# UbiquityRobotics/fiducials

Hardware: AMD Instinct MI355X
Metric: frames/sec @1920x1080 20-marker (aruco detect + pose hot path) (higher is better)
Workload: dtype u8

## Files before the change

fiducials_amd/csrc/fid_api.hip:

```cpp
#include "fid_kernels.hip"

#include <math.h>
#include <stdio.h>
#include <stdlib.h>
#include <string.h>

#include <new>
#include <string>
#include <vector>

namespace {

enum { ST_GRAY = 0, ST_THRESH, ST_STARTS, ST_PROBE, ST_WALK, ST_APPROX, ST_SORT, ST_NEAR, ST_RESOLVE, ST_IDENT, ST_FILTER, ST_SUBPIX, ST_POSE, ST_SEEDWALK,
       ST_SEEDLESS, ST_COUNT };
const char *const kStageNames[ST_COUNT] = {"to_gray", "threshold", "find_starts", "walk_probe", "walk_full", "approx", "sort_cands",
                                           "near", "resolve", "identify", "filter_markers", "subpix", "pose", "seed_walk", "seedless_chain"};

constexpr int TX = 128, TY = 32, NT = 256;
constexpr int THRW_NT = 512, THRW_WT = 16;
static_assert(THRW_NT * THRW_WT >= 8191, "k_threshold_wide: a row per workgroup");

}

struct fid_ctx {
// ... 429 lines not shown
    const int gstride = to_gray ? W : stride;
    const long long gfstride = to_gray ? (long long)W * H : fstride;
    const uint8_t *gray = to_gray ? c->d_gray : d_src;
    set_geometry(c, W, H, gstride, F);
    if (c->wait_ev) {
        HIPCHK(c, hipStreamWaitEvent(st0, c->wait_ev, 0));
        c->wait_ev = nullptr;
    }
    if (c->d_seedhash) {
        if (++c->seed_gen > 1023) {
            HIPCHK(c, hipMemsetAsync(c->d_seedhash, 0, (size_t)c->lim.max_batch * c->seed_hash_cap * sizeof(unsigned long long), st0));
            c->seed_gen = 1;
        }
        c->P.seedGen = c->seed_gen;
    }
    if (c->masks_W != W || c->masks_H != H || c->masks_S != c->P.nscales) {
        HIPCHK(c, hipMemsetAsync(c->d_masks, 0, c->masks_bytes, st0));
        c->masks_W = W;
        c->masks_H = H;
        c->masks_S = c->P.nscales;
    }
    layout_results(c, F);
    if (!c->res_precleared) HIPCHK(c, hipMemsetAsync(c->d_res, 0, c->res_clear_bytes, st0));
    c->res_precleared = false;
    c->piece_chain = c->pieces > 1 && !c->chained && !c->host_feed && !c->from_host_call && !c->whole_border_walk && c->sub_frames <= 0 &&
                     F >= 32 * c->pieces && c->stagger == 0;
    const SubPlan plan = plan_sub_batches(c, F);
    const int nsub = plan.nsub;
    const bool chainp = c->piece_chain;
    c->last_nsub = nsub;
    {
        const fid_status rcs = ensure_streams(c, nsub, F);
        if (rcs != FID_OK) return rcs;
    }
    if (nsub > 1) HIPCHK(c, hipEventRecord(c->fork_ev, st0));
    bool tail_recorded = false;
    auto sub_phase = [&](int sb, int phase) -> fid_status {
        const int f0 = plan.f0[sb], Fs = plan.f0[sb + 1] - f0;
        hipStream_t st = nsub > 1 ? c->sub_stream[chainp ? (sb & 1) : sb] : st0;
        if (nsub > 1 && phase == 0) HIPCHK(c, hipStreamWaitEvent(st, c->fork_ev, 0));
        if (chainp && phase == 0 && sb > 0) HIPCHK(c, hipStreamWaitEvent(st, c->fs_done[sb - 1], 0));
        if (c->host_feed && phase == 0) HIPCHK(c, hipStreamWaitEvent(st, c->in_ready[sb], 0));
        if (nsub > 1 && phase == 0 && c->stagger > 0 && sb >= c->stagger) HIPCHK(c, hipStreamWaitEvent(st, c->walk_done[sb - c->stagger], 0));
        DevParams P = c->P;
        P.nframes = Fs;
        const size_t MC = (size_t)P.maxCands, MM = (size_t)P.maxMarkers;
        const uint8_t *g = gray + (long long)f0 * gfstride;
        uint32_t *masks = c->d_masks + (size_t)f0 * P.nscales * P.TR * P.TC * MT_ROWS;
        uint2 *starts = c->d_starts + (size_t)f0 * P.maxStarts, *surv1 = c->d_surv1 + (size_t)f0 * P.maxStarts,
              *surv = c->d_surv + (size_t)f0 * P.maxStarts;
        uint4 *contours = c->d_contours + (size_t)f0 * P.maxContours;
        uint32_t *tab = c->d_ckpts + (size_t)f0 * 2 * P.maxContours * chunk_tab_pitch(P);
        uint32_t *pool = c->d_pool + (size_t)f0 * P.maxChunks * CKW;
        DevCounts *counts = c->d_counts + f0;
        DevCand *cands = c->d_cands + f0 * MC, *sorted = c->d_sorted + f0 * MC, *filtered = c->d_filtered + f0 * MC;
        uint32_t *nearb = c->d_near + f0 * MC * (MC / 32);
        DevIdent *ident = c->d_ident + f0 * MC;
        fid_marker *pre = c->d_pre + f0 * MM, *markers = c->d_markers + f0 * MM;
        unsigned *worklist = c->d_worklist + f0 * MC, *nwork = c->d_nwork + sb;
        hipEvent_t *ev = c->sub_ev[sb];
        auto mark = [&](int idx) {
            if (c->profile) (void)hipEventRecord(ev[idx], st);
        };
        auto chain_point = [&](int pt) {
            if (sb == nsub - 1 && !tail_recorded && !c->blocking && c->chain_at <= pt) {
                (void)hipEventRecord(c->tail_ev, st);
                tail_recorded = true;
            }
        };
      if (phase == 0) {
        mark(0);
        if (to_gray && (int)enc <= FID_ENC_RGBA8)
            hipLaunchKernelGGL(k_to_gray, dim3(2048), dim3(256), 0, st, d_src + (long long)f0 * fstride, stride, fstride, (int)enc,
                               c->d_gray + (size_t)f0 * W * H, W, H, Fs);
        else if (to_gray)
            hipLaunchKernelGGL(k_raw_to_gray, dim3((W + 255) / 256, (H + 3) / 4, Fs), dim3(64, 4), 0, st, d_src + (long long)f0 * fstride, stride,
                               fstride, (int)enc, c->d_gray + (size_t)f0 * W * H, W, H);
        mark(ST_GRAY + 1);
        {
            bool node_table = P.nscales == 13;
            for (int i = 0; i < P.nscales && node_table; i++) node_table = P.win[i] == 3 + 4 * i;
            if (node_table) {
                const int cols = 64 * c->thr_nw, strips = (W + cols - 1) / cols;
                int RS = c->thr_rows;
                if (RS <= 0) {
                    int segs = (1536 + strips * Fs - 1) / (strips * Fs);
                    const int maxsegs = (H + 63) / 64;
                    segs = segs < 1 ? 1 : (segs > maxsegs ? maxsegs : segs);
                    RS = (H + segs - 1) / segs;
                }
                RS = (RS + 3) & ~3;
                dim3 grid(strips, (H + RS - 1) / RS, Fs);
                if (c->thr_nw == 5 && c->thr_split) launch_thr_stream<5, true>(grid, st, g, gfstride, masks, P, RS, c->thr_xcd);
                else if (c->thr_nw == 5) launch_thr_stream<5, false>(grid, st, g, gfstride, masks, P, RS, c->thr_xcd);
                else if (c->thr_split) launch_thr_stream<3, true>(grid, st, g, gfstride, masks, P, RS, c->thr_xcd);
                else launch_thr_stream<3, false>(grid, st, g, gfstride, masks, P, RS, c->thr_xcd);
            } else if (P.rmax > 40) {
                int bands = (512 + Fs - 1) / Fs;
                const int maxb = (H + 15) / 16;
                bands = bands < 1 ? 1 : (bands > maxb ? maxb : bands);
                const int BH = (H + bands - 1) / bands;
                const size_t lds = (size_t)(W + 1 + THRW_NT / 64) * sizeof(unsigned long long);
                fid_launch_log("k_threshold_wide", THRW_NT, lds);
                hipLaunchKernelGGL((k_threshold_wide<THRW_NT, THRW_WT>), dim3((H + BH - 1) / BH, 1, Fs), dim3(THRW_NT), lds, st, g, gfstride,
                                   masks, P, BH);
            } else {
                int R = P.rmax, RW = TX + 2 * R, RH = TY + 2 * R, PT = (RW + 1) | 1;
                size_t lds = (size_t)(RH + 1) * PT * sizeof(uint32_t);
                dim3 grid((W + TX - 1) / TX, (H + TY - 1) / TY, Fs);
                hipLaunchKernelGGL((k_threshold<TX, TY, NT>), grid, dim3(NT), lds, st, g, gfstride, masks, P);
            }
        }
        mark(ST_THRESH + 1);
      }
        long long k2blocks;
        {
            long long groups = (long long)P.nscales * P.TR * ((P.WW + 15) / 16);
            k2blocks = (groups + 7) / 8;
            if (k2blocks > 256) k2blocks = 256;
        }
      if (phase == 0) {
        if (!c->whole_border_walk) {
            hipLaunchKernelGGL(k_find_starts<true>, dim3((unsigned)k2blocks, Fs), dim3(256), 0, st, masks, starts, counts, c->d_global,
                               c->d_seedq + f0 * (size_t)P.maxContours, P);
            mark(ST_STARTS + 1);
            if (nsub > 1) HIPCHK(c, hipEventRecord(c->fs_done[sb], st));
            chain_point(0);
        }
        return FID_OK;
      }
        if (!c->whole_border_walk && nsub > 1 && c->fs_barrier && !chainp)
            for (int o = 0; o < nsub; o++)
                if (o != sb) HIPCHK(c, hipStreamWaitEvent(st, c->fs_done[o], 0));
        int wb = c->walk_blocks > 0 ? c->walk_blocks : (3072 / WALK_WAVES + Fs - 1) / Fs;
        const int wcap = c->walk_blocks_cap > 0 ? c->walk_blocks_cap : (Fs <= 2 ? 256 : 64);
        wb = wb < 2 ? 2 : (wb > wcap ? wcap : wb);
        const int gm = Fs >= 16 ? 1 : 16 / Fs;
        const int wb2 = wb > 1 ? wb / 2 : 1;
        const int cap1 = pts_cap_first(P);
        const size_t lds1 = k_approx_lds_bytes(cap1);
        const size_t lds2 = k_approx_lds_bytes(P.maxPerim + 1);
        if (c->whole_border_walk) {
            hipLaunchKernelGGL(k_find_starts<false>, dim3((unsigned)k2blocks, Fs), dim3(256), 0, st, masks, starts, counts, c->d_global,
                               (uint2 *)nullptr, P);
            mark(ST_STARTS + 1);
            hipLaunchKernelGGL((k_probe<PROBE0_STEPS, 0>), dim3(64 * gm, Fs), dim3(256), 0, st, masks, starts, surv1, counts, c->d_global, P);
            hipLaunchKernelGGL((k_probe<PROBE1_STEPS, 1>), dim3(16 * gm, Fs), dim3(256), 0, st, masks, surv1, surv, counts, c->d_global, P);
            mark(ST_PROBE + 1);
            hipLaunchKernelGGL(k_walk_full<0>, dim3(wb, Fs), dim3(64 * WALK_WAVES), 0, st, masks, surv, contours, tab, pool, (DevSegC *)nullptr,
                               (DevPend *)nullptr, counts, c->d_global, P);
            mark(ST_WALK + 1);
            fid_launch_log("k_approx", 64, (size_t)(lds1));
            hipLaunchKernelGGL(k_approx, dim3(128 * gm, Fs), dim3(64), lds1, st, contours, tab, pool, cands, counts, P, cap1, 0,
                               (const uint32_t *)nullptr, (const uint32_t *)nullptr);
            fid_launch_log("k_approx", 64, (size_t)(lds2));
            hipLaunchKernelGGL(k_approx, dim3(16 * gm, Fs), dim3(64), lds2, st, contours, tab, pool, cands, counts, P,
                               P.maxPerim + 1, 1, (const uint32_t *)nullptr, (const uint32_t *)nullptr);
            mark(ST_APPROX + 1);
        } else {
            const size_t MCn = (size_t)P.maxContours;
            DevSegC *segs = c->d_segs + f0 * MCn;
            DevPend *pend = c->d_pend + f0 * MCn;
            uint2 *seedq = c->d_seedq + f0 * MCn;
            unsigned long long *seedhash = c->d_seedhash + (size_t)f0 * P.seedHashCap;
            uint4 *wres = c->d_wres + f0 * MCn, *cinfo = c->d_cinfo + f0 * MCn;
            uint32_t *cbase = c->d_cbase + f0 * MCn;
            uint32_t *dense = c->d_dense + (size_t)f0 * P.maxChunks * (CK / 4);
            hipStream_t sa = c->aux_stream[chainp ? (sb & 1) : sb];
            HIPCHK(c, hipEventRecord(c->aux_fork[sb], st));
            HIPCHK(c, hipStreamWaitEvent(sa, c->aux_fork[sb], 0));
            int swb = c->sw_blocks > 0 ? c->sw_blocks : (1024 / SW_WAVES + Fs - 1) / Fs;
            swb = swb < 2 ? 2 : (swb > 4 * wcap ? 4 * wcap : swb);
            uint4 *recs = c->d_recs + 2 * f0 * MCn;
            const int cpb = c->copy_blocks > 0 ? c->copy_blocks : 256;
            if (c->profile) (void)hipEventRecord(ev[14], st);
            hipLaunchKernelGGL(k_seed_walk, dim3(swb, Fs), dim3(64 * SW_WAVES), 0, st, masks, seedq, tab, pool, segs, counts, c->d_global, P);
            if (c->profile) (void)hipEventRecord(ev[15], st);
            mark(ST_PROBE + 1);
            chain_point(1);
            if (c->profile) (void)hipEventRecord(ev[16], sa);
            hipStream_t si = (nsub == 1 && Fs <= 16 && c->idx_stream) ? c->idx_stream : sa;
            if (si != sa) HIPCHK(c, hipStreamWaitEvent(si, c->aux_fork[sb], 0));
            hipLaunchKernelGGL(k_seed_index, dim3(8 * gm, Fs), dim3(256), 0, si, seedq, seedhash, counts, P);
            HIPCHK(c, hipEventRecord(c->aux_idx[sb], si));
            if (c->probe_refill0 && gm == 1)
                hipLaunchKernelGGL((k_probe_refill<PROBE0_STEPS, 0>), dim3(c->probe_refill0, Fs), dim3(256), 0, sa, masks, starts, surv1, counts, c->d_global, P,
                                   (const uint4 *)c->d_probe_tables);
            else
                hipLaunchKernelGGL((k_probe_lut<PROBE0_STEPS, 0>), dim3(64 * gm, Fs), dim3(256), 0, sa, masks, starts, surv1, counts, c->d_global, P,
                                   (const uint4 *)c->d_probe_tables);
            if (c->probe_refill && gm == 1)
                hipLaunchKernelGGL((k_probe_refill<PROBE1_STEPS, 1>), dim3(c->probe_refill, Fs), dim3(256), 0, sa, masks, surv1, surv, counts, c->d_global, P,
                                   (const uint4 *)c->d_probe_tables);
            else
                hipLaunchKernelGGL((k_probe_lut<PROBE1_STEPS, 1>), dim3(16 * gm, Fs), dim3(256), 0, sa, masks, surv1, surv, counts, c->d_global, P,
                                   (const uint4 *)c->d_probe_tables);
            const int wb3 = c->walk2_div > 0 ? (wb / c->walk2_div > 0 ? wb / c->walk2_div : 1) : wb2;
            hipLaunchKernelGGL(k_walk_full<2>, dim3(wb3, Fs), dim3(64 * WALK_WAVES), 0, sa, masks, surv, wres, tab, pool, segs, pend, counts,
                               c->d_global, P);
            if (si != sa) HIPCHK(c, hipStreamWaitEvent(sa, c->aux_idx[sb], 0));
            hipLaunchKernelGGL(k_seg_cycles<0>, dim3(8 * gm, Fs), dim3(64), 0, sa, seedq, segs, pend, wres, contours, cinfo, cbase,
                               recs, counts, c->d_global, P, 1, 0);
            hipLaunchKernelGGL(k_seg_copy, dim3(cpb / 4 > 0 ? cpb / 4 : 1, Fs), dim3(256), 0, sa, recs, tab, pool, dense, counts, P, 1);
            fid_launch_log("k_approx", 64, (size_t)(lds1));
            hipLaunchKernelGGL(k_approx, dim3(32 * gm, Fs), dim3(64), lds1, sa, contours, tab, pool, cands, counts, P, cap1, 0,
                               dense, cbase, 2);
            fid_launch_log("k_approx", 64, (size_t)(lds2));
            hipLaunchKernelGGL(k_approx, dim3(8 * gm, Fs), dim3(64), lds2, sa, contours, tab, pool, cands, counts, P,
                               P.maxPerim + 1, 1, dense, cbase, 2);
            if (c->profile) (void)hipEventRecord(ev[17], sa);
            HIPCHK(c, hipEventRecord(c->aux_join[sb], sa));
            HIPCHK(c, hipStreamWaitEvent(st, c->aux_idx[sb], 0));
            hipLaunchKernelGGL(k_seg_link2, dim3(16 * gm, Fs), dim3(256), 0, st, seedq, segs, seedhash, counts, P);
            const int scb = Fs <= 2 ? (int)((P.maxContours + 63) / 64 < 4096 ? (P.maxContours + 63) / 64 : 4096) : 32 * gm * c->light_x;
            if (Fs <= 2)
                hipLaunchKernelGGL(k_seg_cycles<48>, dim3(scb, Fs), dim3(64), 0, st, seedq, segs, pend, wres, contours, cinfo, cbase,
                                   recs, counts, c->d_global, P, 0, getenv("FID_NO_SEGC_WARM") ? 0 : 1);
            else
                hipLaunchKernelGGL(k_seg_cycles<0>, dim3(scb, Fs), dim3(64), 0, st, seedq, segs, pend, wres, contours, cinfo, cbase,
                                   recs, counts, c->d_global, P, 0, 0);
            hipLaunchKernelGGL(k_seg_copy, dim3(cpb, Fs), dim3(256), 0, st, recs, tab, pool, dense, counts, P, 0);
            mark(ST_WALK + 1);
            chain_point(2);
            fid_launch_log("k_approx", 64, (size_t)(lds1));
            hipLaunchKernelGGL(k_approx, dim3(128 * gm, Fs), dim3(64), lds1, st, contours, tab, pool, cands, counts, P, cap1, 0,
                               dense, cbase, 1);
            fid_launch_log("k_approx", 64, (size_t)(lds2));
            hipLaunchKernelGGL(k_approx, dim3(16 * gm, Fs), dim3(64), lds2, st, contours, tab, pool, cands, counts, P,
                               P.maxPerim + 1, 1, dense, cbase, 1);
            mark(ST_APPROX + 1);
            chain_point(3);
            if (chainp) {
                HIPCHK(c, hipEventRecord(c->front_done[sb], st));
                HIPCHK(c, hipStreamWaitEvent(sa, c->front_done[sb], 0));
                st = sa;
            } else {
                HIPCHK(c, hipStreamWaitEvent(st, c->aux_join[sb], 0));
            }
        }
        if (nsub > 1 && c->stagger > 0) HIPCHK(c, hipEventRecord(c->walk_done[sb], st));
        chain_point(4);
        float4 *cmeta = c->d_cmeta + f0 * MC;
        fid_launch_log("k_sort_cands", 256, (size_t)(MC * 8));
        hipLaunchKernelGGL(k_sort_cands, dim3(Fs, (c->light_x > 1 || Fs < 16) ? 16 : 1), dim3(256), MC * 8, st, cands, sorted, cmeta, counts, P);
        mark(ST_SORT + 1);
        hipLaunchKernelGGL(k_near, dim3(32 * gm * c->light_x, Fs), dim3(256), 0, st, sorted, cmeta, nearb, counts, P);
        mark(ST_NEAR + 1);
        {
            const size_t lds = (size_t)c->resolve_lds_kb * 1024;
            const int near_words = c->resolve_serial ? 0 : (int)((lds - 3 * MC * 4) / 4);
            fid_launch_log("k_resolve", 1024, (size_t)(lds));
            hipLaunchKernelGGL(k_resolve, dim3(Fs), dim3(1024), lds, st, sorted, nearb, filtered, counts, worklist, nwork, P, near_words, c->d_global,
                               c->resolve_reg_max);
        }
        mark(ST_RESOLVE + 1);
        chain_point(5);
        {
            int SZ = (P.markerSize + 2 * P.borderBits) * P.cellSize;
            fid_launch_log("k_identify", 64, (size_t)((size_t)SZ * SZ));
            hipLaunchKernelGGL(k_identify, dim3(c->tail_grid > 0 ? c->tail_grid : 256 * 4), dim3(64), (size_t)SZ * SZ, st, g, gfstride, filtered, worklist, nwork,
                               c->d_dict, ident, c->d_bits + f0 * MC * (size_t)(P.markerSize + 2 * P.borderBits) * (P.markerSize + 2 * P.borderBits), P);
        }
        mark(ST_IDENT + 1);
        fid_launch_log("k_filter_markers", 64, (size_t)((size_t)c->filter_lds * sizeof(fid_marker)));
        hipLaunchKernelGGL(k_filter_markers, dim3(Fs), dim3(64), (size_t)c->filter_lds * sizeof(fid_marker), st, filtered, ident, pre, counts, P,
                           c->d_filter_scratch + f0 * MC, c->filter_lds, c->d_accsrc + f0 * MC, c->d_mksrc + f0 * MM);
        mark(ST_FILTER + 1);
        {
            long long items = (long long)Fs * P.maxMarkers * 4;
            const long long bcap = c->tail_grid > 0 ? 4LL * c->tail_grid : 256 * 16;
            int blocks = (int)(items < bcap ? items : bcap);
            if (P.refine == 2)
                hipLaunchKernelGGL(k_refine_contour, dim3(P.maxMarkers < 64 ? P.maxMarkers : 64, Fs), dim3(64), 0, st, (const fid_marker *)pre, markers,
                                   (const int *)(c->d_mksrc + f0 * MM), (const DevCand *)filtered,
                                   (const uint32_t *)(c->d_dense ? c->d_dense + (size_t)f0 * P.maxChunks * (CK / 4) : nullptr), (const uint32_t *)tab,
                                   (const uint32_t *)pool, counts, P);
            else if (P.subpixWin <= 7)
                hipLaunchKernelGGL(k_subpix<7>, dim3(blocks), dim3(64), 0, st, g, gfstride, pre, markers, counts, c->d_subpix_mask, P);
            else
                hipLaunchKernelGGL(k_subpix<SP_MAXWIN_MAX>, dim3(blocks), dim3(64), 0, st, g, gfstride, pre, markers, counts, c->d_subpix_mask, P);
        }
        mark(ST_SUBPIX + 1);
        if (c->pose_cam_valid) {
            PoseCam cam;
            for (int i = 0; i < 9; i++) cam.K[i] = c->pose_K[i];
            for (int i = 0; i < 5; i++) cam.D[i] = c->pose_D[i];
            cam.fiducial_len = c->pose_len;
            int blocks = (Fs * P.maxMarkers + 7) / 8;
            blocks = blocks < 1 ? 1 : (blocks > 256 * 16 ? 256 * 16 : blocks);
            if (c->profile) (void)hipEventRecord(ev[18], st);
            hipLaunchKernelGGL(k_pose, dim3(blocks), dim3(64), 0, st, (const fid_marker *)markers, (const int *)&counts[0].nmark,
                               (int)(sizeof(DevCounts) / sizeof(int)), (const double *)nullptr, Fs, P.maxMarkers, cam, c->d_poses + f0 * MM);
            if (c->profile) (void)hipEventRecord(ev[19], st);
        }
        chain_point(99);
        if (nsub > 1) {
            HIPCHK(c, hipEventRecord(c->sub_done[sb], st));
            if (!chainp) HIPCHK(c, hipStreamWaitEvent(st0, c->sub_done[sb], 0));
        }
        return FID_OK;
    };
    if (chainp) {
        for (int sb = 0; sb < nsub; sb++)
            for (int phase = 0; phase < 2; phase++) {
                const fid_status rcs = sub_phase(sb, phase);
                if (rcs != FID_OK) return rcs;
            }
        for (int sb = 0; sb < nsub; sb++) HIPCHK(c, hipStreamWaitEvent(st0, c->sub_done[sb], 0));
    } else {
        for (int phase = 0; phase < 2; phase++)
            for (int sb = 0; sb < nsub; sb++) {
                const fid_status rcs = sub_phase(sb, phase);
                if (rcs != FID_OK) return rcs;
            }
    }
    hipStream_t st = st0;
    const DevParams &P = c->P;
    HIPCHK(c, hipGetLastError());
    c->pose_done = false;
    c->map_done = false;
    const bool map_ahead = c->map_n > 0 && c->map_cam_valid;
    if (map_ahead) {
        map_pose_launch(c, st, c->d_markers, &c->d_counts[0].nmark, (int)(sizeof(DevCounts) / sizeof(int)), P.maxMarkers, F, c->map_K, c->map_D, c->d_mposes);
        HIPCHK(c, hipGetLastError());
    }
    HIPCHK(c, hipMemcpyAsync(c->h_res, c->d_res, c->pose_cam_valid ? c->res_poses_end : c->res_markers_end, hipMemcpyDeviceToHost, st));
    if (map_ahead) HIPCHK(c, hipMemcpyAsync(c->h_mposes, c->d_mposes, sizeof(fid_map_pose_out) * (size_t)F, hipMemcpyDeviceToHost, st));
    c->last_frames = F;
    c->last_W = W;
    c->last_H = H;
    c->last_gray = gray;
    c->last_gfstride = gfstride;
    c->pend = {d_src, F, W, H, stride, fstride, enc};
    c->in_flight = true;
    c->chained = false;
    c->wait_ev = nullptr;
    c->wait_copy_ev = nullptr;
    c->fed_from_host = false;
    return FID_OK;
}

fid_status run_detect(fid_ctx *c, const uint8_t *d_src, int F, int W, int H, int stride, long long fstride, fid_encoding enc,
                      fid_marker *out, int cap_per_frame, int *n_per_frame);

fid_status finish_detect(fid_ctx *c, fid_marker *out, int cap_per_frame, int *n_per_frame)
{
    const DevParams &P = c->P;
    const int F = c->pend.F;
    c->in_flight = false;
    HIPCHK(c, hipStreamSynchronize(c->stream));
    c->pose_done = c->pose_cam_valid;
    c->map_done = c->map_n > 0 && c->map_cam_valid;
    if (c->profile) {
        for (int i = 0; i < ST_COUNT; i++) c->stage_ms[i] = 0.f;
        for (int sb = 0; sb < c->last_nsub; sb++)
            for (int i = 0; i <= ST_SUBPIX; i++) {
                float ms = 0.f;
                if (hipEventElapsedTime(&ms, c->sub_ev[sb][i], c->sub_ev[sb][i + 1]) == hipSuccess) c->stage_ms[i] += ms;
            }
        if (!c->whole_border_walk)
            for (int sb = 0; sb < c->last_nsub; sb++) {
                float ms = 0.f;
                if (hipEventElapsedTime(&ms, c->sub_ev[sb][14], c->sub_ev[sb][15]) == hipSuccess) c->stage_ms[ST_SEEDWALK] += ms;
                if (hipEventElapsedTime(&ms, c->sub_ev[sb][16], c->sub_ev[sb][17]) == hipSuccess) c->stage_ms[ST_SEEDLESS] += ms;
                if (c->pose_cam_valid && hipEventElapsedTime(&ms, c->sub_ev[sb][18], c->sub_ev[sb][19]) == hipSuccess) c->stage_ms[ST_POSE] += ms;
            }
    }
#ifdef FID_DEBUG_STATS
    {
        const unsigned long long *d = c->h_global->dbg;
        fprintf(stderr, "walk stats: ranges %llu iters %llu ckpts %llu (forced %llu) active-lanes/iter %.1f cyc/range %.0f ckpt-cyc/range %.0f wait-cyc/range %.0f\n",
                d[7], d[0], d[1], d[5], d[0] ? (double)d[2] / d[0] : 0., d[7] ? (double)d[6] / d[7] : 0., d[7] ? (double)d[3] / d[7] : 0.,
                d[7] ? (double)d[4] / d[7] : 0.);
        fprintf(stderr, "walk waves %llu: total cyc avg %.0f max %llu; own queue dry at avg %.0f max %llu\n", d[12],
                d[12] ? (double)d[8] / d[12] : 0., d[9], d[12] ? (double)d[10] / d[12] : 0., d[11]);
        fprintf(stderr, "walk longest %llu steps, total steps %llu\n", d[13], d[14]);
        fprintf(stderr, "resolve (frame 0, n %llu, %llu label rounds) cycles: load %llu label %llu count %llu components %llu places %llu move %llu\n", d[31] >> 32,
                d[31] & 0xffffffffull, d[25], d[26], d[27], d[28], d[29], d[30]);
        if (d[1])
            fprintf(stderr, "checkpoint cycles: wait %.0f activate %.0f retire %.0f hand-out %.0f chunks %.0f refill %.0f; lanes at a checkpoint: need %.1f loading %.1f final %.1f idle %.1f\n",
                    (double)d[4] / d[1], (double)d[16] / d[1], (double)d[17] / d[1], (double)d[18] / d[1], (double)d[19] / d[1], (double)d[20] / d[1],
                    (double)d[21] / d[1], (double)d[22] / d[1], (double)d[23] / d[1], (double)d[24] / d[1]);
// ... 859 lines not shown
```

fiducials_amd/csrc/fid_kernels.hip:

```cpp
#include <hip/hip_runtime.h>
#include <stdint.h>
#include <float.h>
#include <limits.h>

#include <type_traits>
#include <utility>

#include "fid_device.h"
#include "../../include/fid_abi.h"

#define WAVE 64

__device__ __forceinline__ int lane_id() { return threadIdx.x & (WAVE - 1); }

__device__ __forceinline__ unsigned long long ballot64(int pred) { return __ballot(pred); }

#define FID_DPP(OLD, V, CTRL, RMASK) __builtin_amdgcn_update_dpp((OLD), (V), (CTRL), (RMASK), 0xf, false)
#define FID_DPP_SCAN_STEPS(STEP) STEP(0x111, 0xf) STEP(0x112, 0xf) STEP(0x114, 0xf) STEP(0x118, 0xf) STEP(0x142, 0xa) STEP(0x143, 0xc)

__device__ __forceinline__ int wave_iscan(int v)
{
#define S_(C, M) v += FID_DPP(0, v, C, M);
    FID_DPP_SCAN_STEPS(S_)
#undef S_
// ... 2379 lines not shown
#ifdef FID_DEBUG_STATS
    if (lane == 0) {
        atomicAdd(&G->dbg[0], d_iters);
        atomicAdd(&G->dbg[1], d_ckpts);
        atomicAdd(&G->dbg[2], d_active);
        atomicAdd(&G->dbg[3], d_ckcyc);
        atomicAdd(&G->dbg[6], (unsigned long long)(__builtin_readcyclecounter() - d_t0));
        atomicAdd(&G->dbg[7], 1ull);
        for (int k = 0; k < 4; k++) atomicAdd(&G->dbg[21 + k], d_lanes[k]);
    }
#endif
}

__global__ __launch_bounds__(256) void k_seg_link2(const uint2 *__restrict__ seedq, DevSegC *__restrict__ segs,
                                                    const unsigned long long *__restrict__ seedhash, const DevCounts *__restrict__ counts,
                                                    const DevParams P)
{
    const int f = blockIdx.y;
    unsigned ns = (unsigned)counts[f].nseeds;
    ns = ns < (unsigned)P.maxContours ? ns : (unsigned)P.maxContours;
    const unsigned long long *fsh = seedhash + (long long)f * P.seedHashCap;
    const uint2 *fsq = seedq + (long long)f * P.maxContours;
    DevSegC *fsg = segs + (long long)f * P.maxContours;
    for (unsigned i = blockIdx.x * blockDim.x + threadIdx.x; i < ns; i += gridDim.x * blockDim.x) {
        if (fsg[i].n == SEG_INVALID) continue;
        const unsigned nx = seedhash_find(fsh, P.seedHashCap, P.seedGen, seedhash_key(fsg[i].next_key, (int)(fsq[i].x >> 27)));
        if (nx < ns) {
            fsg[i].next_idx = nx;
            fsg[nx].linked = 1u;
        }
    }
}

template <unsigned SC_HOPS>
__global__ __launch_bounds__(64) void k_seg_cycles(const uint2 *__restrict__ seedq, const DevSegC *__restrict__ segs,
                                                    const DevPend *__restrict__ pend, const uint4 *__restrict__ wres,
                                                    uint4 *__restrict__ contours, uint4 *__restrict__ cinfo, uint32_t *__restrict__ cbase,
                                                    uint4 *__restrict__ recs, DevCounts *__restrict__ counts, DevGlobal *__restrict__ G,
                                                    const DevParams P, int part, int warm)
{
    __shared__ uint2 s_hops[SC_HOPS ? SC_HOPS : 1][SC_HOPS ? 64 : 1];
    const int f = blockIdx.y;
    const int lane = lane_id();
    unsigned ns = (unsigned)counts[f].nseeds, nv = (unsigned)counts[f].nsurv;
    ns = ns < (unsigned)P.maxContours ? ns : (unsigned)P.maxContours;
    nv = nv < (unsigned)P.maxContours ? nv : (unsigned)P.maxContours;
    const unsigned lcap = (unsigned)P.maxContours / 2u, rcap = (unsigned)P.maxContours;
    const uint2 *fsq = seedq + (long long)f * P.maxContours;
    const DevSegC *fsg = segs + (long long)f * P.maxContours;
    const DevPend *fpd = pend + (long long)f * P.maxContours;
    uint4 *fco = contours + (long long)f * P.maxContours + (part ? lcap : 0u);
    uint4 *fci = cinfo + (long long)f * P.maxContours + (part ? lcap : 0u);
    uint32_t *fcb = cbase + (long long)f * P.maxContours + (part ? lcap : 0u);
    uint4 *frc = recs + (long long)f * 2 * P.maxContours + (part ? rcap : 0u);
    unsigned *cnt_slots = (unsigned *)(part ? &counts[f].ncontours2 : &counts[f].ncontours);
    unsigned *cnt_recs = (unsigned *)(part ? &counts[f].nrec2 : &counts[f].nrec);
    const unsigned dcap = (unsigned)P.maxChunks * CK;
    const unsigned W2 = (unsigned)P.W + 2u;
    const unsigned ibeg = part ? ns : 0u, iend = part ? ns + nv : ns;
    if (warm && !part) {
        const unsigned nlines = (ns * (unsigned)sizeof(DevSegC) + 127u) >> 7, nx = (gridDim.x + 7u) >> 3;
        unsigned acc = 0;
        for (unsigned k = (blockIdx.x >> 3) * 64u + (unsigned)lane; k < nlines; k += nx * 64u)
            acc += *reinterpret_cast<const volatile uint32_t *>(reinterpret_cast<const char *>(fsg) + (size_t)k * 128u);
        asm volatile("" ::"v"(acc));
    }
    for (unsigned i0 = ibeg + blockIdx.x * 64; i0 < iend; i0 += gridDim.x * 64) {
        const unsigned i = i0 + lane;
        int accept = 0, hole = 0;
        unsigned L = 0, key = 0, hops = 0, pos = 0, n0 = 0, nx0 = SEG_INVALID;
        uint2 st = make_uint2(0u, 0u);
        if (i < ns) {
            const DevSegC s = fsg[i];
            if (s.n != SEG_INVALID && s.n != 0u && s.linked && (s.ko & s.kh) != 0xffffffffu) {
                bool co = s.ko != 0xffffffffu, ch = s.kh != 0xffffffffu, closed = false;
                unsigned KO = s.ko, KH = s.kh, cur = s.next_idx;
                L = s.n;
                hops = 1;
                while (cur != SEG_INVALID) {
                    if (cur == i) {
                        closed = true;
                        break;
                    }
                    DevSegC r;
                    {
                        const uint4 q = reinterpret_cast<const uint4 *>(fsg + cur)[0];
                        r.next_idx = q.x;
                        r.n = q.y;
                        r.ko = q.z;
                        r.kh = q.w;
                    }
                    if (r.n == SEG_INVALID || r.n == 0u) break;
                    co = co && !(r.ko < s.ko);
                    ch = ch && !(r.kh < s.kh);
                    if (!co && !ch) break;
                    KO = r.ko < KO ? r.ko : KO;
                    KH = r.kh < KH ? r.kh : KH;
                    L += r.n;
                    if (SC_HOPS && hops - 1u < SC_HOPS) s_hops[hops - 1u][lane] = make_uint2(cur, r.n);
                    hops++;
                    if (L > (unsigned)P.maxPerim) break;
                    cur = r.next_idx;
                }
                if (closed && L >= (unsigned)P.minPerim && L <= (unsigned)P.maxPerim) {
                    if (co && KO < KH) {
                        accept = 1;
                        hole = 0;
                        key = s.ko;
                        pos = s.pos & 0xffffu;
                    } else if (ch && KH < KO) {
                        accept = 1;
                        hole = 1;
                        key = s.kh;
                        pos = s.pos >> 16;
                    }
                }
                if (accept) {
                    n0 = s.n;
                    nx0 = s.next_idx;
                    const unsigned ky = key / W2, kx = key - ky * W2;
                    st = make_uint2((kx - 1u - (unsigned)hole) | ((ky - 1u) << 16), (uint32_t)f | ((fsq[i].x >> 27) << 16) | ((uint32_t)hole << 24));
                }
            }
        } else if (i < iend) {
            const unsigned j = i - ns;
            if (!fpd[j].p) {
                const uint4 w = wres[(long long)f * P.maxContours + j];
                if (w.z) {
                    st = make_uint2(w.x, w.y);
                    L = w.z;
                    key = w.w;
                    accept = 2;
                }
            }
        }
        const unsigned long long mk = ballot64(accept);
        if (mk) {
            const unsigned myL = accept ? (L + 7u) & ~7u : 0u, myR = accept == 1 ? hops + 1u : (accept == 2 ? 1u : 0u);
            const unsigned sL = wave_iscan_dpp(myL), sR = wave_iscan_dpp(myR);
            const unsigned totL = (unsigned)__builtin_amdgcn_readlane((int)sL, 63), totR = (unsigned)__builtin_amdgcn_readlane((int)sR, 63);
            unsigned bslot = 0, bdense = 0, brec = 0;
            if (lane == 63) {
                bslot = atomicAdd(cnt_slots, (unsigned)__popcll(mk));
                bdense = atomicAdd((unsigned *)&counts[f].ndense, totL);
                brec = atomicAdd(cnt_recs, totR);
            }
            bslot = (unsigned)__builtin_amdgcn_readlane((int)bslot, 63);
            bdense = (unsigned)__builtin_amdgcn_readlane((int)bdense, 63);
            brec = (unsigned)__builtin_amdgcn_readlane((int)brec, 63);
            const unsigned idx = bslot + (unsigned)__popcll(mk & ((1ull << lane) - 1ull));
            if (accept) {
                if (idx < lcap) {
                    fco[idx] = make_uint4(st.x, st.y, L, key);
                    fci[idx] = make_uint4(i, pos, nx0, 0u);
                    const unsigned dst0 = bdense + sL - myL;
                    unsigned rec = brec + sR - myR;
                    if (dst0 + L > dcap || rec + myR > rcap) {
                        atomicOr(&G->overflow, 8u);
                        fcb[idx] = SEG_INVALID;
                    } else if (accept == 2) {
                        fcb[idx] = dst0;
                        frc[rec] = make_uint4((unsigned)P.maxContours + (i - ns), dst0, L, REC_NO_CHUNK);
                    } else {
                        fcb[idx] = dst0;
                        const unsigned ck0 = fsg[i].chunk0;
                        frc[rec++] = make_uint4(i, dst0, (n0 - pos) | (pos << 16), ck0);
                        unsigned off = n0 - pos, cur = nx0;
                        {
                            const unsigned noted = !SC_HOPS ? 0u : (hops - 1u < SC_HOPS ? hops - 1u : SC_HOPS);
                            for (unsigned h = 0; h < noted; h++) {
                                const uint2 e = s_hops[h][lane];
                                frc[rec++] = make_uint4(e.x, dst0 + off, e.y, fsg[e.x].chunk0);
                                off += e.y;
                                cur = e.x;
                            }
                            if (noted) cur = hops - 1u > noted ? fsg[cur].next_idx : i;
                        }
                        while (cur != i && cur != SEG_INVALID && off < L) {
                            const uint2 q = reinterpret_cast<const uint2 *>(fsg + cur)[0];
                            frc[rec++] = make_uint4(cur, dst0 + off, q.y, fsg[cur].chunk0);
                            off += q.y;
                            cur = q.x;
                        }
                        frc[rec++] = make_uint4(i, dst0 + off, pos, ck0);
                        for (; rec < brec + sR; rec++) frc[rec] = make_uint4(0u, 0u, 0u, 0u);
                    }
                } else {
                    atomicOr(&G->overflow, 2u);
                }
            }
        }
    }
}

#define K4_SHORT_PTS 2048
#define K4_MAX_RAW 9
#define K4_STACK 16
__device__ __host__ inline int pts_cap_first(const DevParams &P) { return P.maxPerim < K4_SHORT_PTS ? P.maxPerim : K4_SHORT_PTS; }
inline size_t k_approx_lds_bytes(int pts_cap) { return (size_t)((pts_cap + 7) & ~7) * sizeof(uint32_t); }

__global__ __launch_bounds__(64) void k_approx(const uint4 *__restrict__ contours, const uint32_t *__restrict__ chunk_tab,
                                                const uint32_t *__restrict__ pool, DevCand *__restrict__ cands,
                                                DevCounts *__restrict__ counts, const DevParams P, int pts_cap, int second_pass,
                                                const uint32_t *__restrict__ dense, const uint32_t *__restrict__ cbase, int part = 0)
{
    extern __shared__ __attribute__((aligned(16))) uint32_t pts[];
    __shared__ int2 stack[K4_STACK];
    __shared__ int dst[2 * 16];
    const int lane = lane_id();
    const int f = blockIdx.y;
    unsigned n = (unsigned)(dense ? (part == 2 ? counts[f].ncontours2 : counts[f].ncontours) : counts[f].nsurv);
    n = n < (unsigned)P.maxStarts ? n : (unsigned)P.maxStarts;
    n = n < (unsigned)P.maxContours ? n : (unsigned)P.maxContours;
    const unsigned loff = part == 2 ? (unsigned)P.maxContours / 2u : 0u;
    if (part) n = n < (unsigned)P.maxContours / 2u ? n : (unsigned)P.maxContours / 2u;
    const int W = P.W, H = P.H;
    const uint4 *fco = contours + (long long)f * P.maxContours + loff;
    const uint32_t *fpool = pool;
    for (unsigned cb = blockIdx.x; cb < n; cb += gridDim.x * 64) {
      const unsigned myci = cb + (unsigned)lane * gridDim.x;
      uint4 mine = make_uint4(0u, 0u, 0u, 0u);
      if (myci < n) mine = fco[myci];
      int take = mine.z != 0;
      if (second_pass) take = take && (int)mine.z > pts_cap_first(P);
      else take = take && (int)mine.z <= pts_cap;
      unsigned long long todo = ballot64(take);
      while (todo) {
        const int src = __ffsll((long long)todo) - 1;
        todo &= todo - 1;
        const unsigned ci = cb + (unsigned)src * gridDim.x;
        uint4 c;
        c.x = (unsigned)__builtin_amdgcn_readlane((int)mine.x, src);
        c.y = (unsigned)__builtin_amdgcn_readlane((int)mine.y, src);
        c.z = (unsigned)__builtin_amdgcn_readlane((int)mine.z, src);
        c.w = (unsigned)__builtin_amdgcn_readlane((int)mine.w, src);
        const int count = (int)c.z;
        const int x0 = c.x & 0xffff, y0 = c.x >> 16;
        const int s = (c.y >> 16) & 0xff, hole = (c.y >> 24) & 1;
        __syncthreads();
        uint32_t pref = 0x80000000u | ci;
        if (dense) {
            const uint32_t cb0 = cbase[(long long)f * P.maxContours + loff + ci];
            if (cb0 == SEG_INVALID) continue;
            pref = cb0;
            const uint8_t *src = reinterpret_cast<const uint8_t *>(dense) + (long long)f * P.maxChunks * CK + cb0;
            uint32_t base = c.x;
            for (int k0 = 0; k0 < count; k0 += 512) {
                const int k = k0 + 8 * lane;
                uint2 w = make_uint2(0u, 0u);
                if (k < count) w = *reinterpret_cast<const uint2 *>(src + k);
                base = codes8_to_points(pts, k, count, base, w);
            }
        } else {
            uint32_t base = c.x;
            for (int k0 = 0; k0 < count; k0 += 512) {
                const int k = k0 + 8 * lane;
                uint32_t w = 0u;
                if (k < count)
                    w = fpool[(long long)chunk_tab[chunk_tab_at(P, f, (unsigned)P.maxContours + ci, (unsigned)k >> 6)] * CKW + ((k & (CK - 1)) >> 3)];
                base = codes8_to_points(pts, k, count, base, codes_nibbles_to_bytes(w));
            }
        }
        __syncthreads();
        double eps = (double)count * P.polyAcc;
        eps *= eps;
        int new_count = 0, reject = 0, top = 0;
        int rs_start = 0, pos = 0, le_eps = 0;
        int sx = 0, sy = 0;
        for (int it = 0; it < 3; it++) {
            pos += rs_start;
            pos = pos >= count ? pos - count : pos;
            uint32_t sp = pts[pos];
            sx = sp & 0xffff;
            sy = sp >> 16;
            unsigned bd = 0, bj = 0;
            {
                int j = 1 + lane, off = pos;
                auto point = [&]() {
                    const uint32_t p = pts[off + j];
                    int dx = (int)(p & 0xffff) - sx, dy = (int)(p >> 16) - sy;
                    unsigned d = (unsigned)(dx * dx + dy * dy);
                    const bool gt = d > bd;
                    bd = gt ? d : bd;
                    bj = gt ? (unsigned)j : bj;
                };
                for (; j < count - pos; j += 64) point();
                off -= count;
                for (; j < count; j += 64) point();
            }
            unsigned md, mj;
            wave_argmax_first(bd, bd ? bj : 0xffffffffu, md, mj);
            if (md > 0) rs_start = (int)mj;
            le_eps = (double)md <= eps;
        }
        if (!le_eps) {
            int2 rs, sl;
            rs.y = sl.x = pos;
            sl.y = rs.x = rs_start + pos >= count ? rs_start + pos - count : rs_start + pos;
            if (lane == 0) {
                stack[0] = rs;
                stack[1] = sl;
            }
            top = 2;
        } else {
            if (lane == 0) {
                dst[0] = sx;
                dst[1] = sy;
            }
            new_count = 1;
        }
        __syncthreads();
        while (top > 0) {
            if (new_count + top > K4_MAX_RAW) {
                reject = 1;
                break;
            }
            int2 sl = stack[--top];
            uint32_t ep = pts[sl.y];
            int ex = ep & 0xffff, ey = ep >> 16;
            uint32_t sp = pts[sl.x];
            sx = sp & 0xffff;
            sy = sp >> 16;
            int mcount = sl.y - sl.x;
            if (mcount < 0) mcount += count;
            mcount -= 1;
            int split = 0;
            if (mcount > 0) {
                int dx = ex - sx, dy = ey - sy;
                unsigned lbd = 0, lbt = 0;
                bool any = false;
                {
                    int t = lane, off = sl.x + 1;
                    auto point = [&]() {
                        const uint32_t p = pts[off + t];
                        int px = p & 0xffff, py = p >> 16;
                        int cr = (py - sy) * dx - (px - sx) * dy;
                        unsigned d = (unsigned)(cr < 0 ? -cr : cr);
                        const bool gt = d > lbd || !any;
                        lbd = gt ? d : lbd;
                        lbt = gt ? (unsigned)t : lbt;
                        any = true;
                    };
                    const int ahead = count - (sl.x + 1) < mcount ? count - (sl.x + 1) : mcount;
                    for (; t < ahead; t += 64) point();
                    off -= count;
                    for (; t < mcount; t += 64) point();
                }
                unsigned mdist, mt;
                wave_argmax_first(any ? lbd : 0u, any ? lbt : 0xffffffffu, mdist, mt);
                double max_dist = (double)mdist;
                int bt = (int)mt;
                le_eps = max_dist * max_dist <= eps * ((double)dx * dx + (double)dy * dy);
                if (!le_eps) {
                    split = sl.x + 1 + bt;
                    split = split >= count ? split - count : split;
                }
            } else {
                le_eps = 1;
            }
            __syncthreads();
            if (le_eps) {
                if (lane == 0) {
                    dst[2 * new_count] = sx;
                    dst[2 * new_count + 1] = sy;
                }
                new_count++;
            } else {
                if (lane == 0) {
                    stack[top] = make_int2(split, sl.y);
                    stack[top + 1] = make_int2(sl.x, split);
                }
                top += 2;
            }
            __syncthreads();
        }
        if (reject || new_count < 4) continue;
        {
            const int cnt = new_count;
            int posd = cnt - 1, wpos, i;
            int spx, spy, ptx, pty, epx, epy;
#define RD(X, Y)                  \
    do {                          \
        X = dst[2 * posd];        \
        Y = dst[2 * posd + 1];    \
        if (++posd >= cnt) posd = 0; \
    } while (0)
            RD(spx, spy);
            wpos = posd;
            RD(ptx, pty);
            for (i = 0; i < cnt && new_count > 2; i++) {
                RD(epx, epy);
                double dx = epx - spx, dy = epy - spy;
                double dist = fabs((double)(ptx - spx) * dy - (double)(pty - spy) * dx);
                double sip = (double)(ptx - spx) * (epx - ptx) + (double)(pty - spy) * (epy - pty);
                __syncthreads();
                if (dist * dist <= 0.5 * eps * (dx * dx + dy * dy) && dx != 0 && dy != 0 && sip >= 0) {
                    new_count--;
                    spx = epx;
                    spy = epy;
                    if (lane == 0) {
                        dst[2 * wpos] = spx;
                        dst[2 * wpos + 1] = spy;
                    }
                    if (++wpos >= cnt) wpos = 0;
                    __syncthreads();
                    RD(ptx, pty);
                    i++;
                    continue;
                }
                spx = ptx;
                spy = pty;
                if (lane == 0) {
// ... 2084 lines not shown
```

Baseline: 38110.

## Gather contour codes directly from segment records in k_approx, skipping dense copy

k_approx now rebuilds each contour's chain codes straight from the segment records and chunk pool into LDS, using per-lane aligned word gathers with atomicOr, instead of reading a dense buffer built by k_seg_copy. The seg_copy launches now run only when refine mode 2 needs the dense buffer. Part-2 contours read a single row via the chunk table. This removes a full copy pass and its global write and read traffic. In exchange k_approx does more complex gathers, LDS atomics and serial loops for long pieces.

```diff
diff --git a/fiducials_amd/csrc/fid_api.hip b/fiducials_amd/csrc/fid_api.hip
--- a/fiducials_amd/csrc/fid_api.hip
+++ b/fiducials_amd/csrc/fid_api.hip
@@ -605,10 +605,10 @@
             mark(ST_WALK + 1);
             fid_launch_log("k_approx", 64, (size_t)(lds1));
             hipLaunchKernelGGL(k_approx, dim3(128 * gm, Fs), dim3(64), lds1, st, contours, tab, pool, cands, counts, P, cap1, 0,
-                               (const uint32_t *)nullptr, (const uint32_t *)nullptr);
+                               (const uint4 *)nullptr, (const uint4 *)nullptr, (const uint32_t *)nullptr);
             fid_launch_log("k_approx", 64, (size_t)(lds2));
             hipLaunchKernelGGL(k_approx, dim3(16 * gm, Fs), dim3(64), lds2, st, contours, tab, pool, cands, counts, P,
-                               P.maxPerim + 1, 1, (const uint32_t *)nullptr, (const uint32_t *)nullptr);
+                               P.maxPerim + 1, 1, (const uint4 *)nullptr, (const uint4 *)nullptr, (const uint32_t *)nullptr);
             mark(ST_APPROX + 1);
         } else {
             const size_t MCn = (size_t)P.maxContours;
@@ -626,6 +626,7 @@
             swb = swb < 2 ? 2 : (swb > 4 * wcap ? 4 * wcap : swb);
             uint4 *recs = c->d_recs + 2 * f0 * MCn;
             const int cpb = c->copy_blocks > 0 ? c->copy_blocks : 256;
+            const bool need_dense = P.refine == 2;
             if (c->profile) (void)hipEventRecord(ev[14], st);
             hipLaunchKernelGGL(k_seed_walk, dim3(swb, Fs), dim3(64 * SW_WAVES), 0, st, masks, seedq, tab, pool, segs, counts, c->d_global, P);
             if (c->profile) (void)hipEventRecord(ev[15], st);
@@ -654,13 +655,14 @@
             if (si != sa) HIPCHK(c, hipStreamWaitEvent(sa, c->aux_idx[sb], 0));
             hipLaunchKernelGGL(k_seg_cycles<0>, dim3(8 * gm, Fs), dim3(64), 0, sa, seedq, segs, pend, wres, contours, cinfo, cbase,
                                recs, counts, c->d_global, P, 1, 0);
-            hipLaunchKernelGGL(k_seg_copy, dim3(cpb / 4 > 0 ? cpb / 4 : 1, Fs), dim3(256), 0, sa, recs, tab, pool, dense, counts, P, 1);
+            if (need_dense)
+                hipLaunchKernelGGL(k_seg_copy, dim3(cpb / 4 > 0 ? cpb / 4 : 1, Fs), dim3(256), 0, sa, recs, tab, pool, dense, counts, P, 1);
             fid_launch_log("k_approx", 64, (size_t)(lds1));
             hipLaunchKernelGGL(k_approx, dim3(32 * gm, Fs), dim3(64), lds1, sa, contours, tab, pool, cands, counts, P, cap1, 0,
-                               dense, cbase, 2);
+                               recs, cinfo, cbase, 2);
             fid_launch_log("k_approx", 64, (size_t)(lds2));
             hipLaunchKernelGGL(k_approx, dim3(8 * gm, Fs), dim3(64), lds2, sa, contours, tab, pool, cands, counts, P,
-                               P.maxPerim + 1, 1, dense, cbase, 2);
+                               P.maxPerim + 1, 1, recs, cinfo, cbase, 2);
             if (c->profile) (void)hipEventRecord(ev[17], sa);
             HIPCHK(c, hipEventRecord(c->aux_join[sb], sa));
             HIPCHK(c, hipStreamWaitEvent(st, c->aux_idx[sb], 0));
@@ -672,15 +674,15 @@
             else
                 hipLaunchKernelGGL(k_seg_cycles<0>, dim3(scb, Fs), dim3(64), 0, st, seedq, segs, pend, wres, contours, cinfo, cbase,
                                    recs, counts, c->d_global, P, 0, 0);
-            hipLaunchKernelGGL(k_seg_copy, dim3(cpb, Fs), dim3(256), 0, st, recs, tab, pool, dense, counts, P, 0);
+            if (need_dense) hipLaunchKernelGGL(k_seg_copy, dim3(cpb, Fs), dim3(256), 0, st, recs, tab, pool, dense, counts, P, 0);
             mark(ST_WALK + 1);
             chain_point(2);
             fid_launch_log("k_approx", 64, (size_t)(lds1));
             hipLaunchKernelGGL(k_approx, dim3(128 * gm, Fs), dim3(64), lds1, st, contours, tab, pool, cands, counts, P, cap1, 0,
-                               dense, cbase, 1);
+                               recs, cinfo, cbase, 1);
             fid_launch_log("k_approx", 64, (size_t)(lds2));
             hipLaunchKernelGGL(k_approx, dim3(16 * gm, Fs), dim3(64), lds2, st, contours, tab, pool, cands, counts, P,
-                               P.maxPerim + 1, 1, dense, cbase, 1);
+                               P.maxPerim + 1, 1, recs, cinfo, cbase, 1);
             mark(ST_APPROX + 1);
             chain_point(3);
             if (chainp) {
diff --git a/fiducials_amd/csrc/fid_kernels.hip b/fiducials_amd/csrc/fid_kernels.hip
--- a/fiducials_amd/csrc/fid_kernels.hip
+++ b/fiducials_amd/csrc/fid_kernels.hip
@@ -2555,9 +2555,9 @@
             if (accept) {
                 if (idx < lcap) {
                     fco[idx] = make_uint4(st.x, st.y, L, key);
-                    fci[idx] = make_uint4(i, pos, nx0, 0u);
                     const unsigned dst0 = bdense + sL - myL;
                     unsigned rec = brec + sR - myR;
+                    fci[idx] = make_uint4(i, pos, nx0, rec);
                     if (dst0 + L > dcap || rec + myR > rcap) {
                         atomicOr(&G->overflow, 8u);
                         fcb[idx] = SEG_INVALID;
@@ -2600,19 +2600,30 @@
 #define K4_MAX_RAW 9
 #define K4_STACK 16
 __device__ __host__ inline int pts_cap_first(const DevParams &P) { return P.maxPerim < K4_SHORT_PTS ? P.maxPerim : K4_SHORT_PTS; }
-inline size_t k_approx_lds_bytes(int pts_cap) { return (size_t)((pts_cap + 7) & ~7) * sizeof(uint32_t); }
+__device__ __host__ inline int k_approx_pts_words(int pts_cap) { return (pts_cap + 7) & ~7; }
+inline size_t k_approx_lds_bytes(int pts_cap) { return (size_t)k_approx_pts_words(pts_cap) * sizeof(uint32_t); }
+__device__ __forceinline__ uint32_t piece_word_mask(int d0, int np, int j)
+{
+    const int lo = d0 - 8 * j, hi = d0 + np - 8 * j;
+    uint32_t m = 0xffffffffu;
+    if (hi < 8) m = (1u << (4 * hi)) - 1u;
+    if (lo > 0) m &= ~((1u << (4 * lo)) - 1u);
+    return m;
+}
+#define K4_LANE_PIECE 64
 
 __global__ __launch_bounds__(64) void k_approx(const uint4 *__restrict__ contours, const uint32_t *__restrict__ chunk_tab,
                                                 const uint32_t *__restrict__ pool, DevCand *__restrict__ cands,
                                                 DevCounts *__restrict__ counts, const DevParams P, int pts_cap, int second_pass,
-                                                const uint32_t *__restrict__ dense, const uint32_t *__restrict__ cbase, int part = 0)
+                                                const uint4 *__restrict__ recs, const uint4 *__restrict__ cinfo,
+                                                const uint32_t *__restrict__ cbase, int part = 0)
 {
     extern __shared__ __attribute__((aligned(16))) uint32_t pts[];
     __shared__ int2 stack[K4_STACK];
     __shared__ int dst[2 * 16];
     const int lane = lane_id();
     const int f = blockIdx.y;
-    unsigned n = (unsigned)(dense ? (part == 2 ? counts[f].ncontours2 : counts[f].ncontours) : counts[f].nsurv);
+    unsigned n = (unsigned)(recs ? (part == 2 ? counts[f].ncontours2 : counts[f].ncontours) : counts[f].nsurv);
     n = n < (unsigned)P.maxStarts ? n : (unsigned)P.maxStarts;
     n = n < (unsigned)P.maxContours ? n : (unsigned)P.maxContours;
     const unsigned loff = part == 2 ? (unsigned)P.maxContours / 2u : 0u;
@@ -2642,25 +2653,86 @@
         const int s = (c.y >> 16) & 0xff, hole = (c.y >> 24) & 1;
         __syncthreads();
         uint32_t pref = 0x80000000u | ci;
-        if (dense) {
+        uint32_t row = (unsigned)P.maxContours + ci;
+        bool whole = true;
+        if (recs) {
             const uint32_t cb0 = cbase[(long long)f * P.maxContours + loff + ci];
             if (cb0 == SEG_INVALID) continue;
             pref = cb0;
-            const uint8_t *src = reinterpret_cast<const uint8_t *>(dense) + (long long)f * P.maxChunks * CK + cb0;
-            uint32_t base = c.x;
-            for (int k0 = 0; k0 < count; k0 += 512) {
-                const int k = k0 + 8 * lane;
-                uint2 w = make_uint2(0u, 0u);
-                if (k < count) w = *reinterpret_cast<const uint2 *>(src + k);
-                base = codes8_to_points(pts, k, count, base, w);
-            }
-        } else {
+            const unsigned rcap = (unsigned)P.maxContours;
+            const uint4 *frc = recs + (long long)f * 2 * P.maxContours + (part == 2 ? rcap : 0u);
+            const unsigned first = cinfo[(long long)f * P.maxContours + loff + ci].w;
+            if (part == 2) {
+                row = frc[first < rcap ? first : 0u].x;
+            } else {
+                whole = false;
+                const int nw = (count + 7) >> 3;
+                uint32_t *codes = pts + k_approx_pts_words(pts_cap) - nw;
+                for (int j = lane; j < nw; j += 64) codes[j] = 0u;
+                __syncthreads();
+                const long long tstride = 2ll * P.maxContours;
+                for (unsigned rb = first, done = 0; done < (unsigned)count && rb < rcap; rb += 64) {
+                    uint4 r = make_uint4(0u, 0u, 0u, 0u);
+                    if (rb + (unsigned)lane < rcap) r = frc[rb + lane];
+                    const unsigned p0 = r.z >> 16;
+                    const unsigned incl = wave_iscan_dpp(r.z & 0xffffu);
+                    const unsigned d0 = done + incl - (r.z & 0xffffu);
+                    const unsigned np = d0 < (unsigned)count ? min(r.z & 0xffffu, (unsigned)count - d0) : 0u;
+                    const bool direct = r.w != REC_NO_CHUNK;
+                    const bool by_lane = np != 0u && np <= K4_LANE_PIECE && direct && p0 + np <= 2 * CK;
+                    const int sh4 = (int)(((p0 - d0) & 7u) * 4u);
+                    if (by_lane) {
+                        const uint32_t *srcw = fpool + (long long)r.w * CKW;
+                        const int swmax = (int)((p0 + np - 1u) >> 3), j1 = (int)((d0 + np - 1u) >> 3);
+                        int sw = ((int)p0 - (int)(d0 & 7u)) >> 3;
+                        uint32_t lo = sw >= 0 ? srcw[sw] : 0u;
+                        for (int j = (int)(d0 >> 3); j <= j1; j++, sw++) {
+                            const uint32_t hi = sw + 1 <= swmax ? srcw[sw + 1] : 0u;
+                            atomicOr(&codes[j], __builtin_amdgcn_alignbit(hi, lo, sh4) & piece_word_mask((int)d0, (int)np, j));
+                            lo = hi;
+                        }
+                    }
+                    unsigned long long longs = ballot64(np != 0u && !by_lane);
+                    while (longs) {
+                        const int pl = __ffsll((long long)longs) - 1;
+                        longs &= longs - 1;
+                        const unsigned prow = (unsigned)__builtin_amdgcn_readlane((int)r.x, pl), pck = (unsigned)__builtin_amdgcn_readlane((int)r.w, pl);
+                        const int pp0 = __builtin_amdgcn_readlane((int)p0, pl), pnp = __builtin_amdgcn_readlane((int)np, pl);
+                        const int pd0 = __builtin_amdgcn_readlane((int)d0, pl), psh4 = __builtin_amdgcn_readlane(sh4, pl);
+                        const uint32_t *trow = chunk_tab + chunk_tab_at(P, f, prow, 0);
+                        const int swmax = (pp0 + pnp - 1) >> 3, j1 = (pd0 + pnp - 1) >> 3;
+                        auto word = [&](int sw) -> uint32_t {
+                            if (sw < 0 || sw > swmax) return 0u;
+                            const unsigned k = (unsigned)sw >> 3;
+                            const uint32_t id = pck != REC_NO_CHUNK && k < 2u ? pck + k : trow[(long long)k * tstride];
+                            return fpool[(long long)id * CKW + (sw & (CKW - 1))];
+                        };
+                        for (int j = (pd0 >> 3) + lane; j <= j1; j += 64) {
+                            const int sw = (pp0 + 8 * j - pd0) >> 3;
+                            atomicOr(&codes[j], __builtin_amdgcn_alignbit(word(sw + 1), word(sw), psh4) & piece_word_mask(pd0, pnp, j));
+                        }
+                    }
+                    const unsigned tot = (unsigned)__builtin_amdgcn_readlane((int)incl, 63);
+                    if (!tot) break;
+                    done += tot;
+                }
+                __syncthreads();
+                uint32_t base = c.x;
+                for (int k0 = 0; k0 < count; k0 += 512) {
+                    const int k = k0 + 8 * lane;
+                    uint32_t w = 0u;
+                    if (k < count) w = codes[k >> 3];
+                    base = codes8_to_points(pts, k, count, base, codes_nibbles_to_bytes(w));
+                }
+            }
+        }
+        if (whole) {
             uint32_t base = c.x;
             for (int k0 = 0; k0 < count; k0 += 512) {
                 const int k = k0 + 8 * lane;
                 uint32_t w = 0u;
                 if (k < count)
-                    w = fpool[(long long)chunk_tab[chunk_tab_at(P, f, (unsigned)P.maxContours + ci, (unsigned)k >> 6)] * CKW + ((k & (CK - 1)) >> 3)];
+                    w = fpool[(long long)chunk_tab[chunk_tab_at(P, f, row, (unsigned)k >> 6)] * CKW + ((k & (CK - 1)) >> 3)];
                 base = codes8_to_points(pts, k, count, base, codes_nibbles_to_bytes(w));
             }
         }
```

Result: slower. 36450 (-4.4%).
